# sjtuytc/UnboundedNeRFPytorch

Measured on NVIDIA H100. Metric: ray-samples/sec (fwd+bwd train step) 8192x512, higher is better.
Workload: dtype f32

## Files before the change

include/ubnerf_b200.h:

```cpp
#ifndef UBNERF_B200_H_
#define UBNERF_B200_H_

#include <stdint.h>

#ifdef __cplusplus
extern "C" {
#endif
#if defined(__GNUC__)
#pragma GCC visibility push(default)
#endif

#define UBN_ABI_VERSION 3

int ubn_abi_version(void);
const char* ubn_last_error_string(void);
int64_t ubn_launch_count(void);
void ubn_reset_launch_count(void);


int ubn_infer_t_minmax(const float* rays_o, const float* rays_d, const float* xyz_min, const float* xyz_max,
                       float near, float far, int64_t n_rays, float* t_min, float* t_max, void* stream);

int ubn_infer_n_samples(const float* rays_d, const float* t_min, const float* t_max, float stepdist,
                        int64_t n_rays, int64_t* n_samples, void* stream);
// ... 248 lines not shown
                      float* h2_save, uint32_t* h1_mask, int single_pass, void* stream);
int ubn_rgbnet_bwd(const float* feat, const int64_t* ray_id, const float* W1k, const float* W2, const float* W3,
                   const float* rgb, const float* h1_save, const float* h2_save, const float* grad_rgb, int64_t n_pts,
                   float* grad_feat, float* grad_view_bias, float* grad_W1k, float* grad_W2, float* grad_b2,
                   float* grad_W3, float* grad_b3, void* stream);

int ubn_rgbnet_bwd_tc_data(const float* W2, const float* W3, const float* rgb, const float* h1_save, const float* h2_save,
                           const float* grad_rgb, int64_t n_pts, float* dz1_out, float* grad_W2, void* stream);
int ubn_rgbnet_bwd_small(const float* feat, const int64_t* ray_id, const float* W1k, const float* W3, const float* rgb,
                         const float* h2_save, const float* grad_rgb, const float* dz1, int64_t n_pts, float* grad_feat,
                         float* grad_view_bias, float* grad_W1k, float* grad_b2, float* grad_W3, float* grad_b3, void* stream);

int ubn_rgbnet_bwd_tc_fused(const float* feat, const int64_t* ray_id, const float* W1k, const float* W2, const float* W3,
                            const float* rgb, const float* h1_save, const float* h2_save, const float* grad_rgb, int64_t n_pts,
                            float* grad_feat, float* grad_view_bias, float* grad_W1k, float* grad_W2, float* grad_b2,
                            float* grad_W3, float* grad_b3, uint32_t* h2_mask_scratch, const uint32_t* h1_mask, int single_pass,
                            void* stream);
int ubn_rgbnet_fwd_tc_k(int n_feat, const float* feat, const float* view_bias, const int64_t* ray_id, const float* W1k,
                        const float* W2, const float* b2, const float* W3, const float* b3, int64_t n_pts, float* rgb, float* h1_save,
                        float* h2_save, uint32_t* h1_mask, int single_pass, void* stream);
int ubn_rgbnet_bwd_tc_fused_k(int n_feat, const float* feat, const int64_t* ray_id, const float* W1k, const float* W2,
                              const float* W3, const float* rgb, const float* h1_save, const float* h2_save, const float* grad_rgb,
                              int64_t n_pts, float* grad_feat, float* grad_view_bias, float* grad_W1k, float* grad_W2, float* grad_b2,
                              float* grad_W3, float* grad_b3, uint32_t* h2_mask_scratch, const uint32_t* h1_mask, int single_pass,
                              void* stream);
int ubn_rgbnet_fwd_tc_kw(int n_feat, int n_hidden, const float* feat, const float* view_bias, const int64_t* ray_id,
                         const float* W1k, const float* W2, const float* b2, const float* W3, const float* b3, int64_t n_pts,
                         float* rgb, float* h1_save, float* h2_save, uint32_t* h1_mask, int single_pass, void* stream);
int ubn_rgbnet_bwd_tc_fused_kw(int n_feat, int n_hidden, const float* feat, const int64_t* ray_id, const float* W1k,
                               const float* W2, const float* W3, const float* rgb, const float* h1_save, const float* h2_save,
                               const float* grad_rgb, int64_t n_pts, float* grad_feat, float* grad_view_bias, float* grad_W1k,
                               float* grad_W2, float* grad_b2, float* grad_W3, float* grad_b3, uint32_t* h2_mask_scratch,
                               const uint32_t* h1_mask, int single_pass, void* stream);

#if defined(__GNUC__)
#pragma GCC visibility pop
#endif
#ifdef __cplusplus
}
#endif
#endif
```

unboundednerfpytorch_b200/_cabi.py:

```python
import ctypes
import os

import torch

_HERE = os.path.dirname(os.path.abspath(__file__))
LIB_PATH = os.path.join(_HERE, 'libubnerf_b200.so')

c_i64 = ctypes.c_int64
c_i32 = ctypes.c_int32
c_int = ctypes.c_int
c_f = ctypes.c_float
c_p = ctypes.c_void_p


class UbnGridDesc(ctypes.Structure):
    _fields_ = [('P', c_i32), ('C', c_i32), ('X', c_i32), ('Y', c_i32), ('Z', c_i32), ('num_freqs', c_i32),
                ('stride_p', c_i64), ('stride_c', c_i64), ('stride_v', c_i64),
                ('xyz_min', c_f * 3), ('xyz_max', c_f * 3)]


class UbnMarchCfg(ctypes.Structure):
    _fields_ = [('scene_center', c_f * 3), ('scene_radius', c_f * 3),
                ('contract_B', c_f), ('contract_A', c_f),
                ('contracted_norm', c_i32), ('n_samples', c_i32),
# ... 14 lines not shown


ABI_VERSION = 3
FLAG_QUERIED, FLAG_LISTED, FLAG_SCANNED, FLAG_KEEP, FLAG_INNER = 1, 2, 4, 8, 16

_SIGNATURES = {
    'ubn_abi_version': [],
    'ubn_last_error_string': [],
    'ubn_launch_count': [],
    'ubn_reset_launch_count': [],
    'ubn_infer_t_minmax': [c_p, c_p, c_p, c_p, c_f, c_f, c_i64, c_p, c_p, c_p],
    'ubn_infer_n_samples': [c_p, c_p, c_p, c_f, c_i64, c_p, c_p],
    'ubn_infer_ray_start_dir': [c_p, c_p, c_p, c_i64, c_p, c_p, c_p],
    'ubn_sample_pts_count': [c_p, c_p, c_p, c_p, c_f, c_f, c_f, c_i64, c_p, c_p, c_p, c_p, c_p, c_p],
    'ubn_sample_pts_emit': [c_p, c_p, c_p, c_p, c_p, c_p, c_f, c_i64, c_i64, c_p, c_p, c_p, c_p, c_p],
    'ubn_sample_ndc_pts_on_rays': [c_p, c_p, c_p, c_p, c_i64, c_i64, c_p, c_p, c_p],
    'ubn_sample_bg_pts_on_rays': [c_p, c_p, c_p, c_f, c_i64, c_i64, c_p, c_p],
    'ubn_maskcache_lookup': [c_p, c_p, c_p, c_p, c_i64, c_i64, c_i64, c_i64, c_p, c_p],
    'ubn_raw2alpha': [c_p, c_f, c_f, c_p, c_i64, c_p, c_p, c_p],
    'ubn_raw2alpha_backward': [c_p, c_p, c_f, c_p, c_i64, c_p, c_p],
    'ubn_alpha2weight': [c_p, c_p, c_i64, c_i64, c_p, c_p, c_p, c_p, c_p, c_p],
    'ubn_alpha2weight_backward': [c_p, c_p, c_p, c_p, c_p, c_p, c_i64, c_i64, c_p, c_p, c_p, c_p],
    'ubn_segment_sum': [c_p, c_i64, c_p, c_i64, c_i64, c_p, c_p, c_p, c_p],
    'ubn_rgbnet_fwd': [c_p] * 8 + [c_i64] + [c_p] * 4,
    'ubn_rgbnet_fwd_tc': [c_p] * 8 + [c_i64] + [c_p] * 4 + [c_int, c_p],
    'ubn_rgbnet_bwd_tc_data': [c_p] * 6 + [c_i64] + [c_p] * 3,
    'ubn_rgbnet_bwd_small': [c_p] * 8 + [c_i64] + [c_p] * 7,
    'ubn_rgbnet_bwd': [c_p] * 9 + [c_i64] + [c_p] * 8,
    'ubn_rgbnet_bwd_tc_fused': [c_p] * 9 + [c_i64] + [c_p] * 9 + [c_int, c_p],
    'ubn_rgbnet_fwd_tc_k': [c_int] + [c_p] * 8 + [c_i64] + [c_p] * 4 + [c_int, c_p],
    'ubn_rgbnet_bwd_tc_fused_k': [c_int] + [c_p] * 9 + [c_i64] + [c_p] * 9 + [c_int, c_p],
    'ubn_rgbnet_fwd_tc_kw': [c_int, c_int] + [c_p] * 8 + [c_i64] + [c_p] * 4 + [c_int, c_p],
    'ubn_rgbnet_bwd_tc_fused_kw': [c_int, c_int] + [c_p] * 9 + [c_i64] + [c_p] * 9 + [c_int, c_p],
    'ubn_total_variation_add_grad': [c_p, c_p, c_f, c_f, c_f, c_i64, c_i64, c_i64, c_i64, c_i64, c_int, c_p],
    'ubn_adam_upd': [c_p, c_p, c_p, c_p, c_p, c_i64, c_int, c_f, c_f, c_f, c_f, c_int, c_p],
    'ubn_tv_adam_fused': [c_p, c_p, c_p, c_p, c_f, c_f, c_f, c_i64, c_i64, c_i64, c_i64, c_i64, c_int, c_int,
                          c_f, c_f, c_f, c_f, c_int, c_int, c_p],
    'ubn_tv_adam_pingpong': [c_p, c_p, c_p, c_p, c_p, c_f, c_f, c_f, c_i64, c_i64, c_i64, c_i64, c_i64, c_int, c_int,
                             c_f, c_f, c_f, c_f, c_int, c_int, c_p],
    'ubn_tv_adam_peer': [c_p, c_p, c_p, c_int, c_p, c_p, c_f, c_f, c_f, c_i64, c_i64, c_i64, c_i64, c_i64, c_int, c_i64, c_i64,
                         c_int, c_f, c_f, c_f, c_f, c_int, c_p],
    'ubn_lattice_alpha': [c_p, ctypes.POINTER(UbnGridDesc), c_p, c_p, c_i64, c_i64, c_i64, c_f, c_f, c_p, c_p],
    'ubn_maxpool3_gt_and': [c_p, c_i64, c_i64, c_i64, c_f, c_p, c_p],
    'ubn_resample_grid': [c_p, ctypes.POINTER(UbnGridDesc), c_p, ctypes.POINTER(UbnGridDesc), c_p],
    'ubn_view_scatter_ones': [c_p, c_p, c_i64, c_i64, c_f, c_f, c_f, ctypes.POINTER(UbnGridDesc), c_p, c_p],
    'ubn_count_gt': [c_p, c_f, c_i64, c_p, c_p],
    'ubn_maskout_near_cam': [c_p, c_i64, c_i64, c_i64, c_i64, c_p, c_i64, c_f, c_f, c_p],
    'ubn_maskout_near_cam_lattice': [c_p, c_i64, c_i64, c_i64, c_i64, c_p, c_p, c_p, c_i64, c_f, c_f, c_p],
    'ubn_cumdist_thres': [c_p, c_f, c_i64, c_i64, c_p, c_p],
    'ubn_get_rays_of_a_view': [c_int, c_int, c_p, c_p, c_int, c_int, c_int, c_int, c_int, c_int, c_p, c_p, c_p, c_p, c_p],
    'ubn_gather_rays': [c_p, c_p, c_int, c_p, c_i64, c_i64, c_p, c_p],
    'ubn_composite_fwd': [c_p, c_p, c_p, c_i64, c_i64, c_p, c_p, c_p, c_p],
    'ubn_composite_bwd': [c_p, c_p, c_p, c_p, c_i64, c_p, c_p, c_p],
    'ubn_distortion_loss': [c_p, c_p, c_p, c_i64, c_i64, c_f, c_p, c_p, c_p, c_p, c_p, c_i64, c_p],
    'ubn_render_loss': [c_p] * 7 + [c_i64, c_i64] + [c_f] * 6 + [c_p] * 6 + [c_i64, c_p],
    'ubn_grid_sample_fwd': [c_p, ctypes.POINTER(UbnGridDesc), c_p, c_i64, c_p, c_p],
    'ubn_grid_sample_bwd': [c_p, ctypes.POINTER(UbnGridDesc), c_p, c_i64, c_p, c_p],
    'ubn_march_density_fwd': [c_p, c_p, c_p, c_p, ctypes.POINTER(UbnGridDesc), c_p, ctypes.POINTER(UbnMarchCfg), c_i64,
                              c_p, c_p, c_p, c_p, c_p, c_p, c_p, c_p],
    'ubn_exclusive_scan_i32': [c_p, c_i64, c_p, c_p, c_p],
    'ubn_march_feature_fwd': [c_p, c_p, c_p, c_p, ctypes.POINTER(UbnGridDesc), ctypes.POINTER(UbnMarchCfg), c_i64,
                              c_p, c_p, c_p, c_p, c_p, c_p, c_p, c_p, c_p, c_p, c_p, c_p, c_p, c_p],
    'ubn_march_feature_fwd_tma': [c_p, c_p, c_p, c_p, ctypes.POINTER(UbnGridDesc), ctypes.POINTER(UbnMarchCfg), c_i64,
                                  c_p, c_p, c_p, c_p, c_p, c_p, c_p, c_p, c_p, c_p, c_p, c_p, c_p, c_p, c_p],
    'ubn_set_feature_kernel': [c_int],
    'ubn_get_feature_kernel': [],
# ... 116 lines not shown
```

unboundednerfpytorch_b200/csrc/common.cuh:

```cuda
#pragma once
#include <cuda_runtime.h>
#include <stdint.h>

#include "../../include/ubnerf_b200.h"

namespace ubn {

constexpr int kNumSMs = 132;

extern thread_local cudaError_t g_last_error;
void count_launch();

inline int finish(cudaError_t e) {
  if (e != cudaSuccess) g_last_error = e;
  return (int)e;
}

inline int after_launch() {
  count_launch();
  return finish(cudaGetLastError());
}

inline cudaStream_t as_stream(void* s) { return reinterpret_cast<cudaStream_t>(s); }

template <typename T>
__host__ __device__ __forceinline__ T ceil_div(T a, T b) { return (a + b - 1) / b; }

inline unsigned blocks_for(int64_t n, int threads) { return (unsigned)((n + threads - 1) / threads); }

__device__ __forceinline__ void ndc_point(float ox, float oy, float oz, float dx, float dy, float dz, int i, int n,
                                          float& x, float& y, float& z) {
  const float dist = __fdiv_rn((float)i, (float)(n - 1));
  x = fmaf(dx, dist, ox);
  y = fmaf(dy, dist, oy);
  z = fmaf(dz, dist, oz);
}

struct RayBox {
  float t_min, t_max;
};

__device__ __forceinline__ RayBox ray_aabb(const float* __restrict__ o, const float* __restrict__ d,
                                           const float* __restrict__ xyz_min,
                                           const float* __restrict__ xyz_max, float near, float far) {
  const float vx = (d[0] == 0) ? (float)1e-6 : d[0];
  const float vy = (d[1] == 0) ? (float)1e-6 : d[1];
  const float vz = (d[2] == 0) ? (float)1e-6 : d[2];
  const float ax = (xyz_max[0] - o[0]) / vx;
  const float ay = (xyz_max[1] - o[1]) / vy;
  const float az = (xyz_max[2] - o[2]) / vz;
  const float bx = (xyz_min[0] - o[0]) / vx;
  const float by = (xyz_min[1] - o[1]) / vy;
  const float bz = (xyz_min[2] - o[2]) / vz;
  RayBox r;
  r.t_min = fmaxf(fminf(fmaxf(fmaxf(fminf(ax, bx), fminf(ay, by)), fminf(az, bz)), far), near);
  r.t_max = fmaxf(fminf(fminf(fminf(fmaxf(ax, bx), fmaxf(ay, by)), fmaxf(az, bz)), far), near);
  return r;
}

__device__ __forceinline__ float ray_norm(const float* __restrict__ d) {
  return sqrtf(d[0] * d[0] + d[1] * d[1] + d[2] * d[2]);
// ... 39 lines not shown
```

unboundednerfpytorch_b200/csrc/render_tma.cu:

```cuda
#include <cuda.h>

#include <algorithm>
#include <cstring>

#include "march_common.cuh"

namespace ubn {

namespace rt {
constexpr int kBox = 8;
constexpr int kChan = 12;
constexpr int kSteps = 4;
constexpr int kSegSteps = 64;
constexpr uint32_t kBoxBytes = kBox * kBox * kBox * kChan * 4;
constexpr int kWarps = 4;
constexpr uint32_t kSmemBytes = kWarps * kBoxBytes + kWarps * 8 + 128;

__device__ __forceinline__ uint32_t smem_u32(const void* p) { return (uint32_t)__cvta_generic_to_shared(p); }

__device__ __forceinline__ void mbar_init(uint32_t bar, uint32_t count) {
  asm volatile("mbarrier.init.shared::cta.b64 [%0], %1;" ::"r"(bar), "r"(count) : "memory");
}
__device__ __forceinline__ void mbar_expect_tx(uint32_t bar, uint32_t bytes) {
  asm volatile("mbarrier.arrive.expect_tx.shared::cta.b64 _, [%0], %1;" ::"r"(bar), "r"(bytes) : "memory");
}
__device__ __forceinline__ void mbar_wait(uint32_t bar, uint32_t parity) {
  asm volatile(
      "{\n\t.reg .pred p;\n\tWAIT_%=:\n\tmbarrier.try_wait.parity.shared::cta.b64 p, [%0], %1;\n\t@p bra DONE_%=;\n\tbra WAIT_%=;\n\t"
      "DONE_%=:\n\t}\n" ::"r"(bar),
      "r"(parity)
      : "memory");
}
__device__ __forceinline__ void tma_load_4d(uint32_t dst, const CUtensorMap* map, uint32_t bar, int c0, int c1, int c2, int c3) {
  asm volatile(
      "cp.async.bulk.tensor.4d.shared::cluster.global.tile.mbarrier::complete_tx::bytes [%0], [%1, {%3, %4, %5, %6}], [%2];" ::"r"(dst),
      "l"(reinterpret_cast<uint64_t>(map)), "r"(bar), "r"(c0), "r"(c1), "r"(c2), "r"(c3)
      : "memory");
}

struct Cell3 {
  int x0, y0, z0;
  float fx, fy, fz;
};

__device__ __forceinline__ Cell3 cell_of(float cx, float cy, float cz, int X, int Y, int Z) {
  Cell3 c;
  const float x0 = fminf(fmaxf(floorf(cx), 0.f), (float)(X - 2));
  const float y0 = fminf(fmaxf(floorf(cy), 0.f), (float)(Y - 2));
  const float z0 = fminf(fmaxf(floorf(cz), 0.f), (float)(Z - 2));
  c.fx = cx - x0; c.fy = cy - y0; c.fz = cz - z0;
  c.x0 = (int)x0; c.y0 = (int)y0; c.z0 = (int)z0;
  return c;
}

__device__ __forceinline__ float cweight(const Cell3& c, int bx, int by, int bz) {
  return ((bz ? c.fz : 1.f - c.fz) * (by ? c.fy : 1.f - c.fy)) * (bx ? c.fx : 1.f - c.fx);
}

}

__global__ void __launch_bounds__(32 * rt::kWarps, 2) k_march_feature_tma(
    const __grid_constant__ CUtensorMap tmap, const float* __restrict__ rays_o, const float* __restrict__ rays_d,
    const float* __restrict__ t_table, GridView g, MarchParams p, int64_t n_rays, const uint8_t* __restrict__ flags,
    const int64_t* __restrict__ offsets, const float* __restrict__ density, const float* __restrict__ alpha,
// ... 178 lines not shown
```

unboundednerfpytorch_b200/csrc/shade_tc.cu:

```cuda
#include <algorithm>

#include "common.cuh"

namespace ubn {
namespace tc {

constexpr int kHidden = 128;
constexpr int kFeat = 12;
constexpr int kUnit = 16;
constexpr int kPanelRows = 128;
__host__ __device__ constexpr int n_tiles(int w) { return w / 8; }
__host__ __device__ constexpr int stride(int w) { return w + 8; }

__host__ __device__ constexpr uint32_t frag_w2(int w) { return n_tiles(w) * n_tiles(w) * 32 * 16; }
__host__ __device__ constexpr uint32_t frag_w1(int w) { return n_tiles(w) * 2 * 32 * 16; }

__device__ __forceinline__ uint32_t tf32_hi_bits(float x) { return __float_as_uint(x) & 0xFFFFE000u; }

__device__ __forceinline__ void mma_tf32(float (&d)[4], const uint32_t (&a)[4], uint32_t b0, uint32_t b1) {
  asm volatile(
      "mma.sync.aligned.m16n8k8.row.col.f32.tf32.tf32.f32 {%0, %1, %2, %3}, {%4, %5, %6, %7}, {%8, %9}, {%0, %1, %2, %3};"
      : "+f"(d[0]), "+f"(d[1]), "+f"(d[2]), "+f"(d[3])
      : "r"(a[0]), "r"(a[1]), "r"(a[2]), "r"(a[3]), "r"(b0), "r"(b1));
}
// ... 742 lines not shown
                           sA[(8 * s + t + 4) * kStride + 16 * mt + g], sA[(8 * s + t + 4) * kStride + 16 * mt + g + 8]};
      uint32_t ah[4], al[4];
      split4(av, ah, al);
#pragma unroll
      for (int j = 0; j < kNT; ++j) {
        const uint2 b0 = sB[(8 * s + t) * kStrideB + 8 * (j0 + j) + g], b1 = sB[(8 * s + t + 4) * kStrideB + 8 * (j0 + j) + g];
        mma3<kThree>(acc[j], ah, al, make_uint4(b0.x, b1.x, b0.y, b1.y));
      }
    }
#pragma unroll
    for (int j = 0; j < kNT; ++j)
#pragma unroll
      for (int e = 0; e < 4; ++e) sum[j][e] += acc[j][e];
  }
#pragma unroll
  for (int j = 0; j < kNT; ++j) {
    const int c = 8 * (j0 + j) + 2 * t, m = 16 * mt + g;
    atomicAdd(grad_W2 + m * kW + c, sum[j][0]);
    atomicAdd(grad_W2 + m * kW + c + 1, sum[j][1]);
    atomicAdd(grad_W2 + (m + 8) * kW + c, sum[j][2]);
    atomicAdd(grad_W2 + (m + 8) * kW + c + 1, sum[j][3]);
  }
}

template <bool kThree, bool kPanel, bool kMask2>
__global__ void __launch_bounds__(dw::kThreads, 1) k_shade_dw2_tc(UBN_SHADE_DW2_PARAMS) {
  shade_dw2_tc<kHidden, kThree, kPanel, kMask2>(UBN_SHADE_DW2_ARGS);
}

template <int kW, bool kThree, int kCtas, bool kPanel, bool kMask2>
__global__ void __launch_bounds__(dw::kThreads, kCtas) k_shade_dw2_tc_w(UBN_SHADE_DW2_PARAMS) {
  shade_dw2_tc<kW, kThree, kPanel, kMask2>(UBN_SHADE_DW2_ARGS);
}
#undef UBN_SHADE_DW2_ARGS
#undef UBN_SHADE_DW2_PARAMS

namespace w64 {
constexpr int kFwdWarps = 8, kFwdCtas = 2;
constexpr int kBwdWarps = 8, kBwdCtas = 1;
constexpr int kDw2Ctas = 2;
}

}
}

using namespace ubn;

namespace {

template <typename K>
int set_smem(K kernel, uint32_t bytes) {
  return finish(cudaFuncSetAttribute(kernel, cudaFuncAttributeMaxDynamicSharedMemorySize, (int)bytes));
}

unsigned unit_grid(int64_t n_pts, int warps, int ctas = 1) {
  const int64_t n_units = (n_pts + tc::kUnit - 1) / tc::kUnit;
  return (unsigned)std::min<int64_t>((int64_t)kNumSMs * ctas, (n_units + warps - 1) / warps);
}

template <int kF, bool kSave, bool kThree, int kWarps, bool kPanel, int kW = tc::kHidden, int kCtas = 1>
int launch_fwd(const float* feat, const float* vb, const int64_t* ray_id, const float* W1k, const float* W2, const float* b2,
               const float* W3, const float* b3, int64_t n, float* rgb, float* h1, float* h2, uint32_t* m1, cudaStream_t st) {
  auto k = [] {
    if constexpr (kW == tc::kHidden) return tc::k_shade_fwd_tc<kF, kSave, kThree, kWarps, kPanel>;
    else return tc::k_shade_fwd_tc_w<kF, kW, kSave, kThree, kWarps, kCtas, kPanel>;
  }();
// ... 16 lines not shown
int launch_bwd(const float* feat, const int64_t* ray_id, const float* W1k, const float* W2, const float* W3, const float* rgb,
               const float* h1, const float* h2, const float* grad_rgb, int64_t n, float* grad_feat, float* grad_vb, float* gW1k,
               float* gb2, float* gW3, float* gb3, uint32_t* m2, const uint32_t* m1, float* dz1, cudaStream_t st) {
  auto k = [] {
    if constexpr (kW != tc::kHidden) {
      static_assert(!kDz1Out, "the dZ1 round trip is a width-128 A/B engine");
      return tc::k_shade_bwd_tc_w<kF, kW, kThree, kWarps, kCtas, kPanel, kMask1>;
    } else if constexpr (kF == tc::kFeat) {
      return tc::k_shade_bwd_tc<kThree, kWarps, kPanel, kMask1, kDz1Out>;
    } else {
      return tc::k_shade_bwd_tc_k<kF, kThree, kWarps, kPanel, kMask1, kDz1Out>;
    }
  }();
  const uint32_t bytes = tc::bk::smem_bytes(kWarps, kF, kW);
  if (int e = set_smem(k, bytes)) return e;
  k<<<unit_grid(n, kWarps, kCtas), 32 * kWarps, bytes, st>>>(feat, ray_id, W1k, W2, W3, rgb, h1, h2, grad_rgb, n, grad_feat, grad_vb, gW1k,
                                                      gb2, gW3, gb3, m2, m1, dz1);
  UBN_LAUNCH_CHECK();
  return 0;
}

template <bool kThree, bool kPanel, bool kMask2, int kW = tc::kHidden, int kCtas = 1>
int launch_dw2(const float* W3, const float* rgb, const float* h1, const float* h2, const uint32_t* m2, const float* grad_rgb,
               int64_t n, float* gW2, cudaStream_t st) {
  auto k = [] {
    if constexpr (kW == tc::kHidden) return tc::k_shade_dw2_tc<kThree, kPanel, kMask2>;
    else return tc::k_shade_dw2_tc_w<kW, kThree, kCtas, kPanel, kMask2>;
  }();
  constexpr uint32_t bytes = tc::dw::smem(kW);
  if (int e = set_smem(k, bytes)) return e;
  const int64_t n_chunks = (n + tc::dw::kK - 1) / tc::dw::kK;
  const unsigned grid = (unsigned)std::min<int64_t>((int64_t)kNumSMs * kCtas, n_chunks);
  k<<<grid, tc::dw::kThreads, bytes, st>>>(W3, rgb, h1, h2, m2, grad_rgb, n, gW2);
  UBN_LAUNCH_CHECK();
  return 0;
}

template <int kF>
int rgbnet_fwd_tc(const float* feat, const float* view_bias, const int64_t* ray_id, const float* W1k, const float* W2, const float* b2,
                  const float* W3, const float* b3, int64_t n_pts, float* rgb, float* h1_save, float* h2_save, uint32_t* h1_mask,
                  int single_pass, void* stream) {
  if (n_pts <= 0) return 0;
  const bool save = h1_save != nullptr && h2_save != nullptr;
  const bool one = (single_pass & 1) != 0, four = (single_pass & 2) != 0, panel = save && (single_pass & 4) != 0;
  cudaStream_t st = as_stream(stream);
#define UBN_FWD(SAVE, THREE, W) \
  return launch_fwd_p<kF, SAVE, THREE, W>(panel, feat, view_bias, ray_id, W1k, W2, b2, W3, b3, n_pts, rgb, h1_save, h2_save, h1_mask, st)
  if (save) {
    if (one) { if (four) UBN_FWD(true, false, 4); else UBN_FWD(true, false, 8); }
    if (four) UBN_FWD(true, true, 4); else UBN_FWD(true, true, 8);
  }
  if (one) { if (four) UBN_FWD(false, false, 4); else UBN_FWD(false, false, 8); }
  if (four) UBN_FWD(false, true, 4); else UBN_FWD(false, true, 8);
#undef UBN_FWD
}

template <int kF>
int rgbnet_bwd_tc_fused(const float* feat, const int64_t* ray_id, const float* W1k, const float* W2, const float* W3, const float* rgb,
                        const float* h1_save, const float* h2_save, const float* grad_rgb, int64_t n_pts, float* grad_feat,
                        float* grad_view_bias, float* grad_W1k, float* grad_W2, float* grad_b2, float* grad_W3, float* grad_b3,
                        uint32_t* h2_mask_scratch, const uint32_t* h1_mask, int single_pass, void* stream) {
  if (n_pts <= 0) return 0;
  cudaStream_t st = as_stream(stream);
  const bool one = (single_pass & 1) != 0, four = (single_pass & 2) != 0 || kF > 12, panel = (single_pass & 4) != 0;
  const bool mask1 = panel && h1_mask != nullptr, mask2 = panel && h2_mask_scratch != nullptr;
  uint32_t* m2 = mask2 ? h2_mask_scratch : nullptr;
  int e = 0;
#define UBN_BWD(THREE, W, P, M1)                                                                                              \
  e = launch_bwd<kF, THREE, W, P, M1, false>(feat, ray_id, W1k, W2, W3, rgb, h1_save, h2_save, grad_rgb, n_pts, grad_feat,        \
                                         grad_view_bias, grad_W1k, grad_b2, grad_W3, grad_b3, m2, h1_mask, nullptr, st)
#define UBN_BWD_W(THREE, P, M1) \
  do { if (four) UBN_BWD(THREE, 4, P, M1); else if constexpr (kF <= 12) UBN_BWD(THREE, 8, P, M1); } while (0)
#define UBN_BWD_T(P, M1) \
  do { if (one) UBN_BWD_W(false, P, M1); else UBN_BWD_W(true, P, M1); } while (0)
  if (mask1) UBN_BWD_T(true, true);
  else if (panel) UBN_BWD_T(true, false);
  else UBN_BWD_T(false, false);
#undef UBN_BWD_T
#undef UBN_BWD_W
#undef UBN_BWD
  if (e) return e;
#define UBN_DW(THREE, P, M2) return launch_dw2<THREE, P, M2>(W3, rgb, h1_save, h2_save, m2, grad_rgb, n_pts, grad_W2, st)
  if (mask2) { if (one) UBN_DW(false, true, true); else UBN_DW(true, true, true); }
  if (panel) { if (one) UBN_DW(false, true, false); else UBN_DW(true, true, false); }
  if (one) UBN_DW(false, false, false); else UBN_DW(true, false, false);
#undef UBN_DW
}

template <int kF, int kW>
int rgbnet_fwd_tc_w(const float* feat, const float* view_bias, const int64_t* ray_id, const float* W1k, const float* W2,
                    const float* b2, const float* W3, const float* b3, int64_t n_pts, float* rgb, float* h1_save, float* h2_save,
                    uint32_t* h1_mask, int single_pass, void* stream) {
  const bool save = h1_save != nullptr && h2_save != nullptr;
  if (save && (single_pass & 4) == 0) return finish(cudaErrorInvalidValue);
  if (n_pts <= 0) return 0;
  const bool one = (single_pass & 1) != 0;
  cudaStream_t st = as_stream(stream);
  constexpr int W = tc::w64::kFwdWarps, C = tc::w64::kFwdCtas;
#define UBN_FWD_W(SAVE, THREE, M1) \
  return launch_fwd<kF, SAVE, THREE, W, SAVE, kW, C>(feat, view_bias, ray_id, W1k, W2, b2, W3, b3, n_pts, rgb, h1_save, h2_save, M1, st)
  if (save) { if (one) UBN_FWD_W(true, false, h1_mask); else UBN_FWD_W(true, true, h1_mask); }
  if (one) UBN_FWD_W(false, false, nullptr); else UBN_FWD_W(false, true, nullptr);
#undef UBN_FWD_W
}

template <int kF, int kW>
int rgbnet_bwd_tc_fused_w(const float* feat, const int64_t* ray_id, const float* W1k, const float* W2, const float* W3,
                          const float* rgb, const float* h1_save, const float* h2_save, const float* grad_rgb, int64_t n_pts,
                          float* grad_feat, float* grad_view_bias, float* grad_W1k, float* grad_W2, float* grad_b2, float* grad_W3,
                          float* grad_b3, uint32_t* h2_mask_scratch, const uint32_t* h1_mask, int single_pass, void* stream) {
  if ((single_pass & 4) == 0 || h1_mask == nullptr || h2_mask_scratch == nullptr) return finish(cudaErrorInvalidValue);
  if (n_pts <= 0) return 0;
  const bool one = (single_pass & 1) != 0;
  cudaStream_t st = as_stream(stream);
  constexpr int W = tc::w64::kBwdWarps, C = tc::w64::kBwdCtas, C2 = tc::w64::kDw2Ctas;
#define UBN_BWD_W(THREE)                                                                                                        \
  launch_bwd<kF, THREE, W, true, true, false, kW, C>(feat, ray_id, W1k, W2, W3, rgb, h1_save, h2_save, grad_rgb, n_pts, grad_feat, \
                                                     grad_view_bias, grad_W1k, grad_b2, grad_W3, grad_b3, h2_mask_scratch, h1_mask,  \
                                                     nullptr, st)
  if (int e = one ? UBN_BWD_W(false) : UBN_BWD_W(true)) return e;
#undef UBN_BWD_W
  if (one) return launch_dw2<false, true, true, kW, C2>(W3, rgb, h1_save, h2_save, h2_mask_scratch, grad_rgb, n_pts, grad_W2, st);
  return launch_dw2<true, true, true, kW, C2>(W3, rgb, h1_save, h2_save, h2_mask_scratch, grad_rgb, n_pts, grad_W2, st);
}

}

extern "C" int ubn_rgbnet_fwd_tc(const float* feat, const float* view_bias, const int64_t* ray_id, const float* W1k,
                                 const float* W2, const float* b2, const float* W3, const float* b3, int64_t n_pts,
                                 float* rgb, float* h1_save, float* h2_save, uint32_t* h1_mask, int single_pass, void* stream) {
  return rgbnet_fwd_tc<tc::kFeat>(feat, view_bias, ray_id, W1k, W2, b2, W3, b3, n_pts, rgb, h1_save, h2_save, h1_mask, single_pass,
                                  stream);
}

extern "C" int ubn_rgbnet_fwd_tc_k(int n_feat, const float* feat, const float* view_bias, const int64_t* ray_id, const float* W1k,
                                   const float* W2, const float* b2, const float* W3, const float* b3, int64_t n_pts, float* rgb,
                                   float* h1_save, float* h2_save, uint32_t* h1_mask, int single_pass, void* stream) {
#define UBN_FWD_K(F) \
  return rgbnet_fwd_tc<F>(feat, view_bias, ray_id, W1k, W2, b2, W3, b3, n_pts, rgb, h1_save, h2_save, h1_mask, single_pass, stream)
  switch (n_feat) {
    case 3: UBN_FWD_K(3);
    case 12: UBN_FWD_K(12);
    case 15: UBN_FWD_K(15);
    default: return finish(cudaErrorInvalidValue);
  }
#undef UBN_FWD_K
}

extern "C" int ubn_rgbnet_bwd_tc_data(const float* W2, const float* W3, const float* rgb, const float* h1_save,
                                      const float* h2_save, const float* grad_rgb, int64_t n_pts, float* dz1_out,
                                      float* grad_W2, void* stream) {
  if (n_pts <= 0) return 0;
  cudaStream_t st = as_stream(stream);
  if (int e = launch_bwd<tc::kFeat, true, 8, false, false, true>(nullptr, nullptr, nullptr, W2, W3, rgb, h1_save, h2_save, grad_rgb, n_pts,
                                                     nullptr, nullptr, nullptr, nullptr, nullptr, nullptr, nullptr, nullptr,
                                                     dz1_out, st))
    return e;
  return launch_dw2<true, false, false>(W3, rgb, h1_save, h2_save, nullptr, grad_rgb, n_pts, grad_W2, st);
}

// ... 53 lines not shown
```

unboundednerfpytorch_b200/ops.py:

```python
import ctypes

import torch

from . import _cabi
from ._cabi import c_f, c_i64, c_int, check, ptr, stream_of


def _chk(x, name, dtype=torch.float32, contiguous=True):
    if not isinstance(x, torch.Tensor) or not x.is_cuda:
        raise RuntimeError(f'{name} must be a CUDA tensor')
    if contiguous and not x.is_contiguous():
        raise RuntimeError(f'{name} must be contiguous')
    if dtype is not None and x.dtype != dtype:
        raise RuntimeError(f'{name} must be {dtype} (got {x.dtype})')
    return x


def _scalar(v):
    return float(v)


class _Guard:

    def __init__(self, t):
# ... 356 lines not shown
        raise RuntimeError('slab must be a dense [X,Y,Z] view')
    cams = cams.contiguous().float()
    with _Guard(slab) as lib:
        if lattice is None:
            check(lib.ubn_maskout_near_cam(ptr(slab), c_i64(sv), c_i64(X), c_i64(Y), c_i64(Z), ptr(cams), c_i64(cams.shape[0]),
                                           c_f(float(near_clip)), c_f(float(fill)), stream_of(slab)))
        else:
            lo, hi = ((c_f * 3)(*[float(v) for v in b]) for b in lattice)
            check(lib.ubn_maskout_near_cam_lattice(ptr(slab), c_i64(sv), c_i64(X), c_i64(Y), c_i64(Z), lo, hi, ptr(cams),
                                                   c_i64(cams.shape[0]), c_f(float(near_clip)), c_f(float(fill)), stream_of(slab)))
    return slab


def set_feature_kernel(variant):
    from ._cabi import load
    check(load().ubn_set_feature_kernel(c_int(int(variant))))


def get_feature_kernel():
    from ._cabi import load
    return int(load().ubn_get_feature_kernel())


def set_density_scatter(variant):
    from ._cabi import load
    check(load().ubn_set_density_scatter(c_int(int(variant))))


def get_density_scatter():
    from ._cabi import load
    return int(load().ubn_get_density_scatter())


def cumdist_thres(dist, thres):
    _chk(dist, 'dist')
    mask = torch.empty(dist.shape, dtype=torch.bool, device=dist.device)
    if dist.numel() == 0:
        return mask
    with _Guard(dist) as lib:
        check(lib.ubn_cumdist_thres(ptr(dist), c_f(float(thres)), c_i64(dist.shape[0]), c_i64(dist.shape[1]), ptr(mask),
                                    stream_of(dist)))
    return mask
```

Measured before the change: 151.2 million.

## Add warp-specialized WGMMA kernel for rgbnet grad_W2 with cp.async producer pipeline

Adds a new Hopper kernel for the W2 weight-gradient reduction. A producer warpgroup stages h1 tiles into 128B-swizzled shared memory through a multi-stage mbarrier ring, fed by cp.async. Two consumer warpgroups compute the masked dh in registers and issue wgmma m64n128k8 TF32, including a 3-pass hi/lo split for precision, then atomically add the result into grad_W2. It is the default when the h2 mask path is in use and is meant to replace the mma.sync dw2 kernel. The cost is one CTA per SM, more complexity, and a per-chunk wait on wgmma completion, which limits overlap.

```diff
diff --git a/include/ubnerf_b200.h b/include/ubnerf_b200.h
--- a/include/ubnerf_b200.h
+++ b/include/ubnerf_b200.h
@@ -304,6 +304,7 @@
                                const float* grad_rgb, int64_t n_pts, float* grad_feat, float* grad_view_bias, float* grad_W1k,
                                float* grad_W2, float* grad_b2, float* grad_W3, float* grad_b3, uint32_t* h2_mask_scratch,
                                const uint32_t* h1_mask, int single_pass, void* stream);
+int ubn_set_dw2_engine(int engine);
 
 #if defined(__GNUC__)
 #pragma GCC visibility pop
diff --git a/unboundednerfpytorch_b200/_cabi.py b/unboundednerfpytorch_b200/_cabi.py
--- a/unboundednerfpytorch_b200/_cabi.py
+++ b/unboundednerfpytorch_b200/_cabi.py
@@ -70,6 +70,7 @@
     'ubn_rgbnet_bwd_tc_fused_k': [c_int] + [c_p] * 9 + [c_i64] + [c_p] * 9 + [c_int, c_p],
     'ubn_rgbnet_fwd_tc_kw': [c_int, c_int] + [c_p] * 8 + [c_i64] + [c_p] * 4 + [c_int, c_p],
     'ubn_rgbnet_bwd_tc_fused_kw': [c_int, c_int] + [c_p] * 9 + [c_i64] + [c_p] * 9 + [c_int, c_p],
+    'ubn_set_dw2_engine': [c_int],
     'ubn_total_variation_add_grad': [c_p, c_p, c_f, c_f, c_f, c_i64, c_i64, c_i64, c_i64, c_i64, c_int, c_p],
     'ubn_adam_upd': [c_p, c_p, c_p, c_p, c_p, c_i64, c_int, c_f, c_f, c_f, c_f, c_int, c_p],
     'ubn_tv_adam_fused': [c_p, c_p, c_p, c_p, c_f, c_f, c_f, c_i64, c_i64, c_i64, c_i64, c_i64, c_int, c_int,
diff --git a/unboundednerfpytorch_b200/csrc/common.cuh b/unboundednerfpytorch_b200/csrc/common.cuh
--- a/unboundednerfpytorch_b200/csrc/common.cuh
+++ b/unboundednerfpytorch_b200/csrc/common.cuh
@@ -27,6 +27,22 @@
 __host__ __device__ __forceinline__ T ceil_div(T a, T b) { return (a + b - 1) / b; }
 
 inline unsigned blocks_for(int64_t n, int threads) { return (unsigned)((n + threads - 1) / threads); }
+
+__device__ __forceinline__ uint32_t smem_u32(const void* p) { return (uint32_t)__cvta_generic_to_shared(p); }
+
+__device__ __forceinline__ void mbar_init(uint32_t bar, uint32_t count) {
+  asm volatile("mbarrier.init.shared::cta.b64 [%0], %1;" ::"r"(bar), "r"(count) : "memory");
+}
+__device__ __forceinline__ void mbar_arrive(uint32_t bar) {
+  asm volatile("mbarrier.arrive.shared::cta.b64 _, [%0];" ::"r"(bar) : "memory");
+}
+__device__ __forceinline__ void mbar_wait(uint32_t bar, uint32_t parity) {
+  asm volatile(
+      "{\n\t.reg .pred p;\n\tWAIT_%=:\n\tmbarrier.try_wait.parity.shared::cta.b64 p, [%0], %1;\n\t@p bra DONE_%=;\n\tbra WAIT_%=;\n\t"
+      "DONE_%=:\n\t}\n" ::"r"(bar),
+      "r"(parity)
+      : "memory");
+}
 
 __device__ __forceinline__ void ndc_point(float ox, float oy, float oz, float dx, float dy, float dz, int i, int n,
                                           float& x, float& y, float& z) {
diff --git a/unboundednerfpytorch_b200/csrc/render_tma.cu b/unboundednerfpytorch_b200/csrc/render_tma.cu
--- a/unboundednerfpytorch_b200/csrc/render_tma.cu
+++ b/unboundednerfpytorch_b200/csrc/render_tma.cu
@@ -16,20 +16,8 @@
 constexpr int kWarps = 4;
 constexpr uint32_t kSmemBytes = kWarps * kBoxBytes + kWarps * 8 + 128;
 
-__device__ __forceinline__ uint32_t smem_u32(const void* p) { return (uint32_t)__cvta_generic_to_shared(p); }
-
-__device__ __forceinline__ void mbar_init(uint32_t bar, uint32_t count) {
-  asm volatile("mbarrier.init.shared::cta.b64 [%0], %1;" ::"r"(bar), "r"(count) : "memory");
-}
 __device__ __forceinline__ void mbar_expect_tx(uint32_t bar, uint32_t bytes) {
   asm volatile("mbarrier.arrive.expect_tx.shared::cta.b64 _, [%0], %1;" ::"r"(bar), "r"(bytes) : "memory");
-}
-__device__ __forceinline__ void mbar_wait(uint32_t bar, uint32_t parity) {
-  asm volatile(
-      "{\n\t.reg .pred p;\n\tWAIT_%=:\n\tmbarrier.try_wait.parity.shared::cta.b64 p, [%0], %1;\n\t@p bra DONE_%=;\n\tbra WAIT_%=;\n\t"
-      "DONE_%=:\n\t}\n" ::"r"(bar),
-      "r"(parity)
-      : "memory");
 }
 __device__ __forceinline__ void tma_load_4d(uint32_t dst, const CUtensorMap* map, uint32_t bar, int c0, int c1, int c2, int c3) {
   asm volatile(
diff --git a/unboundednerfpytorch_b200/csrc/shade_tc.cu b/unboundednerfpytorch_b200/csrc/shade_tc.cu
--- a/unboundednerfpytorch_b200/csrc/shade_tc.cu
+++ b/unboundednerfpytorch_b200/csrc/shade_tc.cu
@@ -798,6 +798,213 @@
 __global__ void __launch_bounds__(dw::kThreads, kCtas) k_shade_dw2_tc_w(UBN_SHADE_DW2_PARAMS) {
   shade_dw2_tc<kW, kThree, kPanel, kMask2>(UBN_SHADE_DW2_ARGS);
 }
+
+namespace wg {
+constexpr int kThreads = 384;
+constexpr int kStages = 4;
+constexpr int kProducerRegs = 80, kConsumerRegs = 208;
+constexpr uint32_t kTile = kHidden * dw::kK * 4;
+constexpr uint32_t kExtra = 1024;
+__host__ __device__ constexpr uint32_t stage_bytes(bool three) { return (three ? 2 : 1) * kTile + kExtra; }
+constexpr int kRaw = 3;
+constexpr uint32_t kRawH1 = 8 * 128 * 16;
+constexpr uint32_t kRawSlot = kRawH1 + 2 * 6 * 32 * 4;
+__host__ __device__ constexpr uint32_t oRaw(bool three) { return kStages * stage_bytes(three); }
+__host__ __device__ constexpr uint32_t oBar(bool three) { return oRaw(three) + kRaw * kRawSlot; }
+__host__ __device__ constexpr uint32_t smem(bool three) { return oBar(three) + 2 * kStages * 8 + 1024; }
+}
+
+__device__ __forceinline__ uint32_t sw128_off(int n, int k) { return n * 128 + ((((k >> 2) ^ n) & 7) << 4) + (k & 3) * 4; }
+
+__device__ __forceinline__ uint64_t sw128_desc(uint32_t addr) {
+  return (uint64_t)((addr & 0x3FFFF) >> 4) | (1ull << 16) | ((uint64_t)(1024 >> 4) << 32) | (1ull << 62);
+}
+
+template <int kScaleD>
+__device__ __forceinline__ void wgmma_tf32(float (&d)[64], const uint32_t (&a)[4], uint64_t desc) {
+  asm volatile(
+      "{\n\t.reg .pred p;\n\tsetp.ne.b32 p, %69, 0;\n\t"
+      "wgmma.mma_async.sync.aligned.m64n128k8.f32.tf32.tf32 "
+      "{%0, %1, %2, %3, %4, %5, %6, %7, %8, %9, %10, %11, %12, %13, %14, %15, %16, %17, %18, %19, %20, %21, %22, %23, %24, %25, "
+      "%26, %27, %28, %29, %30, %31, %32, %33, %34, %35, %36, %37, %38, %39, %40, %41, %42, %43, %44, %45, %46, %47, %48, %49, %50, "
+      "%51, %52, %53, %54, %55, %56, %57, %58, %59, %60, %61, %62, %63}, {%64, %65, %66, %67}, %68, p, 1, 1;\n\t}\n"
+      : "+f"(d[0]), "+f"(d[1]), "+f"(d[2]), "+f"(d[3]), "+f"(d[4]), "+f"(d[5]), "+f"(d[6]), "+f"(d[7]), "+f"(d[8]), "+f"(d[9]),
+        "+f"(d[10]), "+f"(d[11]), "+f"(d[12]), "+f"(d[13]), "+f"(d[14]), "+f"(d[15]), "+f"(d[16]), "+f"(d[17]), "+f"(d[18]),
+        "+f"(d[19]), "+f"(d[20]), "+f"(d[21]), "+f"(d[22]), "+f"(d[23]), "+f"(d[24]), "+f"(d[25]), "+f"(d[26]), "+f"(d[27]),
+        "+f"(d[28]), "+f"(d[29]), "+f"(d[30]), "+f"(d[31]), "+f"(d[32]), "+f"(d[33]), "+f"(d[34]), "+f"(d[35]), "+f"(d[36]),
+        "+f"(d[37]), "+f"(d[38]), "+f"(d[39]), "+f"(d[40]), "+f"(d[41]), "+f"(d[42]), "+f"(d[43]), "+f"(d[44]), "+f"(d[45]),
+        "+f"(d[46]), "+f"(d[47]), "+f"(d[48]), "+f"(d[49]), "+f"(d[50]), "+f"(d[51]), "+f"(d[52]), "+f"(d[53]), "+f"(d[54]),
+        "+f"(d[55]), "+f"(d[56]), "+f"(d[57]), "+f"(d[58]), "+f"(d[59]), "+f"(d[60]), "+f"(d[61]), "+f"(d[62]), "+f"(d[63])
+      : "r"(a[0]), "r"(a[1]), "r"(a[2]), "r"(a[3]), "l"(desc), "n"(kScaleD));
+}
+
+__device__ __forceinline__ void cp_async16(uint32_t dst, const void* src, bool ok) {
+  asm volatile("cp.async.cg.shared.global [%0], [%1], 16, %2;" ::"r"(dst), "l"(src), "r"(ok ? 16 : 0) : "memory");
+}
+__device__ __forceinline__ void cp_async4(uint32_t dst, const void* src, bool ok) {
+  asm volatile("cp.async.ca.shared.global [%0], [%1], 4, %2;" ::"r"(dst), "l"(src), "r"(ok ? 4 : 0) : "memory");
+}
+
+__device__ __forceinline__ void dw2_raw_issue(uint8_t* slot, const float* __restrict__ rgb, const float* __restrict__ h1_save,
+                                              const uint32_t* __restrict__ h2_mask, const float* __restrict__ grad_rgb,
+                                              int64_t ch, int64_t n_chunks, int64_t n_pts, int tid) {
+  const int pw = tid >> 5, lane = tid & 31;
+  if (ch < n_chunks) {
+    const int64_t r = ch * dw::kK + lane;
+    const bool ok = r < n_pts;
+    const float* src = h1_save + (ok ? save_idx<true, kHidden>(r, 4 * pw) : 0);
+    const uint32_t dst = smem_u32(slot) + tid * 16;
+#pragma unroll
+    for (int j = 0; j < 8; ++j) cp_async16(dst + j * 128 * 16, ok ? src + j * 4 * kPanelRows * 4 : h1_save, ok);
+    const uint32_t xd = smem_u32(slot + wg::kRawH1) + (pw * 6 * 32 + lane) * 4;
+    if (pw == 0) {
+#pragma unroll
+      for (int i = 0; i < 3; ++i) {
+        cp_async4(xd + i * 128, ok ? rgb + r * 3 + i : rgb, ok);
+        cp_async4(xd + (3 + i) * 128, ok ? grad_rgb + r * 3 + i : grad_rgb, ok);
+      }
+    } else if (pw == 1) {
+#pragma unroll
+      for (int c = 0; c < kHidden / 32; ++c) cp_async4(xd + c * 128, ok ? h2_mask + mask_idx<kHidden>(r, c) : h2_mask, ok);
+    }
+  }
+  asm volatile("cp.async.commit_group;" ::: "memory");
+}
+
+template <bool kThree>
+__device__ __forceinline__ void dw2_stage_put(const uint8_t* slot, uint8_t* stage, int tid) {
+  const int pw = tid >> 5, lane = tid & 31;
+  const float4* h1 = reinterpret_cast<const float4*>(slot);
+#pragma unroll
+  for (int j = 0; j < 8; ++j) {
+    const int q = pw + 4 * j;
+    const float4 h = h1[j * 128 + tid];
+    const float v[4] = {h.x, h.y, h.z, h.w};
+    uint32_t hi[4], lo[4];
+    split4(v, hi, lo);
+#pragma unroll
+    for (int e = 0; e < 4; ++e) {
+      const uint32_t off = sw128_off(4 * q + e, lane);
+      *reinterpret_cast<uint32_t*>(stage + off) = hi[e];
+      if (kThree) *reinterpret_cast<uint32_t*>(stage + wg::kTile + off) = lo[e];
+    }
+  }
+  const float* x = reinterpret_cast<const float*>(slot + wg::kRawH1) + pw * 6 * 32 + lane;
+  float* sx = reinterpret_cast<float*>(stage + (kThree ? 2 : 1) * wg::kTile) + lane;
+  if (pw == 0) {
+#pragma unroll
+    for (int i = 0; i < 3; ++i) sx[i * 32] = x[(3 + i) * 32] * x[i * 32] * (1.f - x[i * 32]);
+  } else if (pw == 1) {
+#pragma unroll
+    for (int c = 0; c < kHidden / 32; ++c) sx[(3 + c) * 32] = x[c * 32];
+  }
+}
+
+template <bool kThree>
+__global__ void __launch_bounds__(wg::kThreads, 1) k_shade_dw2_wgmma(const float* __restrict__ W3, const float* __restrict__ rgb,
+                                                                      const float* __restrict__ h1_save,
+                                                                      const uint32_t* __restrict__ h2_mask,
+                                                                      const float* __restrict__ grad_rgb, int64_t n_pts,
+                                                                      float* __restrict__ grad_W2) {
+  constexpr int kW = kHidden;
+  constexpr uint32_t kStage = wg::stage_bytes(kThree);
+  extern __shared__ __align__(16) uint8_t smem_raw[];
+  uint8_t* smem = reinterpret_cast<uint8_t*>((reinterpret_cast<uintptr_t>(smem_raw) + 1023) & ~(uintptr_t)1023);
+  const int tid = threadIdx.x, lane = tid & 31;
+  const uint32_t full0 = smem_u32(smem + wg::oBar(kThree)), empty0 = full0 + 8 * wg::kStages;
+  if (tid == 0) {
+    for (int s = 0; s < wg::kStages; ++s) {
+      mbar_init(full0 + 8 * s, 128);
+      mbar_init(empty0 + 8 * s, 256);
+    }
+  }
+  __syncthreads();
+  const int64_t n_chunks = (n_pts + dw::kK - 1) / dw::kK, step = gridDim.x;
+
+  if (tid < 128) {
+    asm volatile("setmaxnreg.dec.sync.aligned.u32 %0;\n" ::"n"(wg::kProducerRegs));
+    uint8_t* raw = smem + wg::oRaw(kThree);
+    const int64_t ch0 = blockIdx.x;
+    for (int k = 0; k < wg::kRaw - 1; ++k)
+      dw2_raw_issue(raw + k * wg::kRawSlot, rgb, h1_save, h2_mask, grad_rgb, ch0 + k * step, n_chunks, n_pts, tid);
+    int i = 0;
+    for (int64_t ch = ch0; ch < n_chunks; ch += step, ++i) {
+      dw2_raw_issue(raw + (i + wg::kRaw - 1) % wg::kRaw * wg::kRawSlot, rgb, h1_save, h2_mask, grad_rgb,
+                    ch + (wg::kRaw - 1) * step, n_chunks, n_pts, tid);
+      asm volatile("cp.async.wait_group %0;" ::"n"(wg::kRaw - 1) : "memory");
+      const int s = i % wg::kStages;
+      mbar_wait(empty0 + 8 * s, ((i / wg::kStages) & 1) ^ 1);
+      dw2_stage_put<kThree>(raw + i % wg::kRaw * wg::kRawSlot, smem + s * kStage, tid);
+      asm volatile("fence.proxy.async.shared::cta;" ::: "memory");
+      mbar_arrive(full0 + 8 * s);
+    }
+    return;
+  }
+
+  asm volatile("setmaxnreg.inc.sync.aligned.u32 %0;\n" ::"n"(wg::kConsumerRegs));
+  const int ct = tid - 128, g = lane >> 2, t = lane & 3;
+  const int m0 = 64 * (ct >> 7) + 16 * ((ct >> 5) & 3) + g;
+  float w3[3][2];
+#pragma unroll
+  for (int i = 0; i < 3; ++i) {
+    w3[i][0] = W3[i * kW + m0];
+    w3[i][1] = W3[i * kW + m0 + 8];
+  }
+  float acc[64], sum[64];
+#pragma unroll
+  for (int e = 0; e < 64; ++e) acc[e] = sum[e] = 0.f;
+  int i = 0;
+  for (int64_t ch = blockIdx.x; ch < n_chunks; ch += step, ++i) {
+    const int s = i % wg::kStages;
+    mbar_wait(full0 + 8 * s, (i / wg::kStages) & 1);
+    uint8_t* stage = smem + s * kStage;
+    const float* sx = reinterpret_cast<const float*>(stage + (kThree ? 2 : 1) * wg::kTile);
+    uint32_t ah[4][4], al[4][4];
+#pragma unroll
+    for (int ks = 0; ks < dw::kK / 8; ++ks) {
+      float av[4];
+#pragma unroll
+      for (int q = 0; q < 2; ++q) {
+        const int k = 8 * ks + t + 4 * q;
+        const float dz3[3] = {sx[k], sx[32 + k], sx[64 + k]};
+        const uint32_t w = __float_as_uint(sx[(3 + (m0 >> 5)) * 32 + k]) >> (m0 & 31);
+#pragma unroll
+        for (int h = 0; h < 2; ++h) {
+          const float dh = dz3[0] * w3[0][h] + dz3[1] * w3[1][h] + dz3[2] * w3[2][h];
+          av[2 * q + h] = ((w >> (8 * h)) & 1u) ? dh : 0.f;
+        }
+      }
+      split4(av, ah[ks], al[ks]);
+    }
+    const uint32_t b = smem_u32(stage);
+    asm volatile("wgmma.fence.sync.aligned;" ::: "memory");
+#pragma unroll
+    for (int ks = 0; ks < dw::kK / 8; ++ks) {
+      const uint64_t bh = sw128_desc(b + 32 * ks);
+      if (kThree) {
+        if (ks == 0) wgmma_tf32<0>(acc, al[ks], bh);
+        else wgmma_tf32<1>(acc, al[ks], bh);
+        wgmma_tf32<1>(acc, ah[ks], sw128_desc(b + wg::kTile + 32 * ks));
+        wgmma_tf32<1>(acc, ah[ks], bh);
+      } else if (ks == 0) {
+        wgmma_tf32<0>(acc, ah[ks], bh);
+      } else {
+        wgmma_tf32<1>(acc, ah[ks], bh);
+      }
+    }
+    asm volatile("wgmma.commit_group.sync.aligned;" ::: "memory");
+    asm volatile("wgmma.wait_group.sync.aligned 0;" ::: "memory");
+#pragma unroll
+    for (int e = 0; e < 64; ++e) asm volatile("" : "+f"(acc[e])::"memory");
+    mbar_arrive(empty0 + 8 * s);
+#pragma unroll
+    for (int e = 0; e < 64; ++e) sum[e] += acc[e];
+  }
+#pragma unroll
+  for (int j = 0; j < 16; ++j)
+#pragma unroll
+    for (int e = 0; e < 4; ++e) atomicAdd(grad_W2 + (m0 + 8 * (e >> 1)) * kW + 8 * j + 2 * t + (e & 1), sum[4 * j + e]);
+}
 #undef UBN_SHADE_DW2_ARGS
 #undef UBN_SHADE_DW2_PARAMS
 
@@ -880,6 +1087,20 @@
   const int64_t n_chunks = (n + tc::dw::kK - 1) / tc::dw::kK;
   const unsigned grid = (unsigned)std::min<int64_t>((int64_t)kNumSMs * kCtas, n_chunks);
   k<<<grid, tc::dw::kThreads, bytes, st>>>(W3, rgb, h1, h2, m2, grad_rgb, n, gW2);
+  UBN_LAUNCH_CHECK();
+  return 0;
+}
+
+int g_dw2_engine = 1;
+
+template <bool kThree>
+int launch_dw2_wgmma(const float* W3, const float* rgb, const float* h1, const uint32_t* m2, const float* grad_rgb, int64_t n,
+                     float* gW2, cudaStream_t st) {
+  auto k = tc::k_shade_dw2_wgmma<kThree>;
+  constexpr uint32_t bytes = tc::wg::smem(kThree);
+  if (int e = set_smem(k, bytes)) return e;
+  const int64_t n_chunks = (n + tc::dw::kK - 1) / tc::dw::kK;
+  k<<<(unsigned)std::min<int64_t>(kNumSMs, n_chunks), tc::wg::kThreads, bytes, st>>>(W3, rgb, h1, m2, grad_rgb, n, gW2);
   UBN_LAUNCH_CHECK();
   return 0;
 }
@@ -929,6 +1150,10 @@
 #undef UBN_BWD
   if (e) return e;
 #define UBN_DW(THREE, P, M2) return launch_dw2<THREE, P, M2>(W3, rgb, h1_save, h2_save, m2, grad_rgb, n_pts, grad_W2, st)
+  if (mask2 && g_dw2_engine == 1) {
+    if (one) return launch_dw2_wgmma<false>(W3, rgb, h1_save, m2, grad_rgb, n_pts, grad_W2, st);
+    return launch_dw2_wgmma<true>(W3, rgb, h1_save, m2, grad_rgb, n_pts, grad_W2, st);
+  }
   if (mask2) { if (one) UBN_DW(false, true, true); else UBN_DW(true, true, true); }
   if (panel) { if (one) UBN_DW(false, true, false); else UBN_DW(true, true, false); }
   if (one) UBN_DW(false, false, false); else UBN_DW(true, false, false);
@@ -974,6 +1199,12 @@
 
 }
 
+extern "C" int ubn_set_dw2_engine(int engine) {
+  if (engine < 0 || engine > 1) return finish(cudaErrorInvalidValue);
+  g_dw2_engine = engine;
+  return 0;
+}
+
 extern "C" int ubn_rgbnet_fwd_tc(const float* feat, const float* view_bias, const int64_t* ray_id, const float* W1k,
                                  const float* W2, const float* b2, const float* W3, const float* b3, int64_t n_pts,
                                  float* rgb, float* h1_save, float* h2_save, uint32_t* h1_mask, int single_pass, void* stream) {
diff --git a/unboundednerfpytorch_b200/ops.py b/unboundednerfpytorch_b200/ops.py
--- a/unboundednerfpytorch_b200/ops.py
+++ b/unboundednerfpytorch_b200/ops.py
@@ -412,6 +412,11 @@
     return int(load().ubn_get_density_scatter())
 
 
+def set_dw2_engine(engine):
+    from ._cabi import load
+    check(load().ubn_set_dw2_engine(c_int(int(engine))))
+
+
 def cumdist_thres(dist, thres):
     _chk(dist, 'dist')
     mask = torch.empty(dist.shape, dtype=torch.bool, device=dist.device)
```

After: 160.8 million, median of 6. 1.06x the previous value.
